# Coder-Yu/QRec

Hardware: AMD Instinct MI355X
Metric: BPR triplet-updates/sec (higher is better)
Workload: dtype f32

## Files before the change

qrec_amd/csrc/reduce.hip:

```cpp
#include "common.h"

using namespace qrec;

namespace {

template <typename T, typename V4>
__global__ __launch_bounds__(256) void sumsq_kernel(const T *__restrict__ x, int64_t n_elems,
                                                    double *__restrict__ out) {
    double acc = 0.0;
    const int64_t n4 = n_elems >> 2;
    const V4 *x4 = reinterpret_cast<const V4 *>(x);
    for (int64_t k = (int64_t)blockIdx.x * blockDim.x + threadIdx.x; k < n4;
         k += (int64_t)gridDim.x * blockDim.x) {
        const V4 v = x4[k];
        acc += (double)v.x * v.x + (double)v.y * v.y + (double)v.z * v.z + (double)v.w * v.w;
    }
    if (blockIdx.x == 0 && threadIdx.x < (n_elems & 3)) {
        const double v = (double)x[(n4 << 2) + threadIdx.x];
        acc += v * v;
    }
#pragma unroll
    for (int m = 32; m >= 1; m >>= 1) acc += __shfl_xor(acc, m, kWave);
    __shared__ double s_part[4];
    if ((threadIdx.x & 63) == 0) s_part[threadIdx.x >> 6] = acc;
    __syncthreads();
    if (threadIdx.x == 0) atomicAdd(out, s_part[0] + s_part[1] + s_part[2] + s_part[3]);
}

__device__ inline void driver_decide(double *__restrict__ stats, double *__restrict__ state, double regU, double regI,
                                     double max_lr, double tol, double *__restrict__ log, int64_t log_capacity) {
    const double nll = atomicAdd(stats + 0, 0.0);
    const double tp = stats[1], tq = stats[2];
    const double loss = nll + regU * tp + regI * tq;
    const double last = state[QREC_DRV_LAST_LOSS], lr_used = state[QREC_DRV_LR];
    const int64_t epoch = (int64_t)state[QREC_DRV_EPOCHS] + 1;
    double lr = lr_used;
    const bool finite = loss == loss && fabs(loss) <= 1.79769313486231570e308;
    const bool converged = finite && fabs(last - loss) < tol;
    if (finite && !converged) {
        if (epoch > 1) lr *= fabs(last) > fabs(loss) ? 1.05 : 0.5;
        if (max_lr > 0.0 && lr > max_lr) lr = max_lr;
    }
    state[QREC_DRV_LR] = lr;
    state[QREC_DRV_LAST_LOSS] = loss;
    state[QREC_DRV_EPOCHS] = (double)epoch;
    state[QREC_DRV_CONVERGED] = converged ? 1.0 : 0.0;
    state[QREC_DRV_FAILED] = finite ? 0.0 : 1.0;
    if (log && epoch <= log_capacity) {
        double *e = log + (epoch - 1) * QREC_DRV_LOG_WORDS;
        e[0] = loss; e[1] = lr_used; e[2] = nll; e[3] = last - loss; e[4] = tp; e[5] = tq;
    }
    stats[0] = 0.0;
}

template <typename T, typename V4>
__device__ inline double block_sumsq(const T *__restrict__ x, int64_t n_elems, double *s_part) {
    double acc = 0.0;
    const int64_t n4 = n_elems >> 2;
    const V4 *x4 = reinterpret_cast<const V4 *>(x);
    for (int64_t k = (int64_t)blockIdx.x * blockDim.x + threadIdx.x; k < n4; k += (int64_t)gridDim.x * blockDim.x) {
        const V4 v = x4[k];
        acc += (double)v.x * v.x + (double)v.y * v.y + (double)v.z * v.z + (double)v.w * v.w;
    }
#pragma unroll
    for (int m = 32; m >= 1; m >>= 1) acc += __shfl_xor(acc, m, kWave);
    __syncthreads();
    if ((threadIdx.x & 63) == 0) s_part[threadIdx.x >> 6] = acc;
    __syncthreads();
    return s_part[0] + s_part[1] + s_part[2] + s_part[3];
}

template <typename T, typename V4>
__global__ __launch_bounds__(256) void epoch_close_kernel(const T *__restrict__ P, int64_t p_elems,
                                                          const T *__restrict__ Q, int64_t q_elems,
                                                          double *__restrict__ stats, double *__restrict__ state,
                                                          double regU, double regI, double max_lr, double tol,
                                                          double *__restrict__ log, int64_t log_capacity, int decide) {
    if (state && (state[QREC_DRV_CONVERGED] != 0.0 || state[QREC_DRV_FAILED] != 0.0)) return;
    __shared__ double s_part[4];
    __shared__ bool s_last;
    const double sp = block_sumsq<T, V4>(P, p_elems, s_part);
    const double sq = block_sumsq<T, V4>(Q, q_elems, s_part);
    double *part = stats + QREC_STATS_PARTIALS;
    unsigned int *ticket = reinterpret_cast<unsigned int *>(stats + 3);
    if (threadIdx.x == 0) {
        __hip_atomic_store(part + 2 * blockIdx.x, sp, __ATOMIC_RELAXED, __HIP_MEMORY_SCOPE_AGENT);
        __hip_atomic_store(part + 2 * blockIdx.x + 1, sq, __ATOMIC_RELAXED, __HIP_MEMORY_SCOPE_AGENT);
        __threadfence();
        s_last = atomicAdd(ticket, 1u) == gridDim.x - 1;
    }
    __syncthreads();
    if (!s_last) return;
    __threadfence();
    double tp = 0.0, tq = 0.0;
    for (unsigned b = threadIdx.x; b < gridDim.x; b += blockDim.x) {
        tp += __hip_atomic_load(part + 2 * b, __ATOMIC_RELAXED, __HIP_MEMORY_SCOPE_AGENT);
        tq += __hip_atomic_load(part + 2 * b + 1, __ATOMIC_RELAXED, __HIP_MEMORY_SCOPE_AGENT);
    }
#pragma unroll
    for (int m = 32; m >= 1; m >>= 1) { tp += __shfl_xor(tp, m, kWave); tq += __shfl_xor(tq, m, kWave); }
    __shared__ double s_tot[2][4];
    if ((threadIdx.x & 63) == 0) { s_tot[0][threadIdx.x >> 6] = tp; s_tot[1][threadIdx.x >> 6] = tq; }
    __syncthreads();
    if (threadIdx.x != 0) return;
    tp = s_tot[0][0] + s_tot[0][1] + s_tot[0][2] + s_tot[0][3];
    tq = s_tot[1][0] + s_tot[1][1] + s_tot[1][2] + s_tot[1][3];
    if (!(decide & 2)) stats[1] = tp;
    if (!(decide & 4)) stats[2] = tq;
    *ticket = 0u;
    if (decide & 1) driver_decide(stats, state, regU, regI, max_lr, tol, log, log_capacity);
}

__global__ void epoch_decide_kernel(double *__restrict__ stats, double *__restrict__ state, double regU, double regI,
                                    double max_lr, double tol, double *__restrict__ log, int64_t log_capacity) {
    if (state[QREC_DRV_CONVERGED] != 0.0 || state[QREC_DRV_FAILED] != 0.0) return;
    driver_decide(stats, state, regU, regI, max_lr, tol, log, log_capacity);
}


__device__ inline bool last_block_total(double mine, int lane_of_pair, double *__restrict__ stats, double *total) {
    __shared__ bool s_last;
    __shared__ double s_tot[4];
    double *part = stats + QREC_STATS_PARTIALS;
    unsigned int *ticket = reinterpret_cast<unsigned int *>(stats + 3);
    if (threadIdx.x == 0) {
        __hip_atomic_store(part + 2 * blockIdx.x + lane_of_pair, mine, __ATOMIC_RELAXED, __HIP_MEMORY_SCOPE_AGENT);
        __threadfence();
        s_last = atomicAdd(ticket, 1u) == gridDim.x - 1;
    }
    __syncthreads();
    if (!s_last) return false;
    __threadfence();
    double t = 0.0;
    for (unsigned b = threadIdx.x; b < gridDim.x; b += blockDim.x)
        t += __hip_atomic_load(part + 2 * b + lane_of_pair, __ATOMIC_RELAXED, __HIP_MEMORY_SCOPE_AGENT);
#pragma unroll
    for (int m = 32; m >= 1; m >>= 1) t += __shfl_xor(t, m, kWave);
    if ((threadIdx.x & 63) == 0) s_tot[threadIdx.x >> 6] = t;
    __syncthreads();
    if (threadIdx.x != 0) return false;
    *total = s_tot[0] + s_tot[1] + s_tot[2] + s_tot[3];
    *ticket = 0u;
    return true;
}

__global__ __launch_bounds__(256) void dist_pre_kernel(const float *__restrict__ P, int64_t p_elems, const float4 *__restrict__ Q,
                                                       const float4 *__restrict__ start, float4 *__restrict__ delta,
                                                       int64_t q4, double *__restrict__ stats, const double *__restrict__ state) {
    if (state && (state[QREC_DRV_CONVERGED] != 0.0 || state[QREC_DRV_FAILED] != 0.0)) return;
    __shared__ double s_part[4];
    for (int64_t k = (int64_t)blockIdx.x * blockDim.x + threadIdx.x; k < q4; k += (int64_t)gridDim.x * blockDim.x) {
        const float4 a = Q[k], b = start[k];
        delta[k] = make_float4(a.x - b.x, a.y - b.y, a.z - b.z, a.w - b.w);
    }
    const double sp = block_sumsq<float, float4>(P, p_elems, s_part);
    double total;
    if (last_block_total(sp, 0, stats, &total)) stats[1] = total;
}

__global__ __launch_bounds__(256) void dist_post_kernel(float4 *__restrict__ Q, float4 *__restrict__ start,
                                                        const float4 *__restrict__ delta, int64_t q4, double *__restrict__ stats,
                                                        double *__restrict__ state, double regU, double regI, double max_lr,
                                                        double tol, double *__restrict__ log, int64_t log_capacity) {
    if (state[QREC_DRV_CONVERGED] != 0.0 || state[QREC_DRV_FAILED] != 0.0) return;
    double acc = 0.0;
    for (int64_t k = (int64_t)blockIdx.x * blockDim.x + threadIdx.x; k < q4; k += (int64_t)gridDim.x * blockDim.x) {
        const float4 s = start[k], d = delta[k];
        const float4 r = make_float4(s.x + d.x, s.y + d.y, s.z + d.z, s.w + d.w);
        start[k] = r;
        Q[k] = r;
        acc += (double)r.x * r.x + (double)r.y * r.y + (double)r.z * r.z + (double)r.w * r.w;
    }
#pragma unroll
    for (int m = 32; m >= 1; m >>= 1) acc += __shfl_xor(acc, m, kWave);
    __shared__ double s_part[4];
    if ((threadIdx.x & 63) == 0) s_part[threadIdx.x >> 6] = acc;
    __syncthreads();
    const double sq = s_part[0] + s_part[1] + s_part[2] + s_part[3];
    double total;
    if (last_block_total(sq, 1, stats, &total)) {
        stats[2] = total;
        driver_decide(stats, state, regU, regI, max_lr, tol, log, log_capacity);
    }
}

}

namespace {
int launch_epoch_close(const void *d_P, int64_t p_rows, const void *d_Q, int64_t q_rows, int dtype, int32_t ld,
                       double *d_stats, double *d_state, double regU, double regI, double max_lr, double tol,
                       double *d_log, int64_t log_capacity, int decide, hipStream_t st) {
    const int64_t pe = p_rows * (int64_t)ld, qe = q_rows * (int64_t)ld;
    int64_t blocks = ((pe > qe ? pe : qe) / 4 + 255) / 256;
    if (blocks > QREC_STATS_MAX_BLOCKS) blocks = QREC_STATS_MAX_BLOCKS;
    if (blocks < 1) blocks = 1;
    if (dtype == QREC_F32)
        hipLaunchKernelGGL((epoch_close_kernel<float, float4>), dim3((unsigned)blocks), dim3(256), 0, st, (const float *)d_P, pe,
                           (const float *)d_Q, qe, d_stats, d_state, regU, regI, max_lr, tol, d_log, log_capacity, decide);
    else
        hipLaunchKernelGGL((epoch_close_kernel<double, double4>), dim3((unsigned)blocks), dim3(256), 0, st, (const double *)d_P, pe,
                           (const double *)d_Q, qe, d_stats, d_state, regU, regI, max_lr, tol, d_log, log_capacity, decide);
    QREC_LAUNCH_CHECK();
    return QREC_OK;
}
}

extern "C" int qrec_epoch_close(const void *d_P, int64_t p_rows, const void *d_Q, int64_t q_rows, int dtype, int32_t ld,
                                double *d_stats, double *d_state, double regU, double regI, double max_lr,
                                double tol, double *d_log, int64_t log_capacity, void *stream) {
    QREC_REQUIRE(d_P && d_Q && d_stats && d_state && p_rows >= 0 && q_rows >= 0 && ld >= 4 && ld % 4 == 0,
                 "qrec_epoch_close: bad arguments");
    QREC_REQUIRE(dtype == QREC_F32 || dtype == QREC_F64, "qrec_epoch_close: bad dtype %d", dtype);
    QREC_REQUIRE(log_capacity == 0 || d_log, "qrec_epoch_close: log capacity without a log");
    return launch_epoch_close(d_P, p_rows, d_Q, q_rows, dtype, ld, d_stats, d_state, regU, regI, max_lr, tol, d_log,
                              log_capacity, 1, as_stream(stream));
}

extern "C" int qrec_epoch_sums(const void *d_P, int64_t p_rows, const void *d_Q, int64_t q_rows, int dtype, int32_t ld,
                               double *d_stats, const double *d_state, void *stream) {
    QREC_REQUIRE(d_P && d_Q && d_stats && p_rows >= 0 && q_rows >= 0 && ld >= 4 && ld % 4 == 0, "qrec_epoch_sums: bad arguments");
    QREC_REQUIRE(dtype == QREC_F32 || dtype == QREC_F64, "qrec_epoch_sums: bad dtype %d", dtype);
    return launch_epoch_close(d_P, p_rows, d_Q, q_rows, dtype, ld, d_stats, const_cast<double *>(d_state), 0, 0, 0, 0,
                              nullptr, 0, 0, as_stream(stream));
}
extern "C" int qrec_epoch_sum_table(const void *d_X, int64_t rows, int dtype, int32_t ld, double *d_stats, int slot,
                                    const double *d_state, void *stream) {
    QREC_REQUIRE(d_X && d_stats && rows >= 0 && ld >= 4 && ld % 4 == 0, "qrec_epoch_sum_table: bad arguments");
    QREC_REQUIRE(dtype == QREC_F32 || dtype == QREC_F64, "qrec_epoch_sum_table: bad dtype %d", dtype);
    QREC_REQUIRE(slot == 1 || slot == 2, "qrec_epoch_sum_table: slot must be 1 (sum P*P) or 2 (sum Q*Q)");
    return slot == 1 ? launch_epoch_close(d_X, rows, d_X, 0, dtype, ld, d_stats, const_cast<double *>(d_state), 0, 0, 0, 0, nullptr,
                                          0, 4, as_stream(stream))
                     : launch_epoch_close(d_X, 0, d_X, rows, dtype, ld, d_stats, const_cast<double *>(d_state), 0, 0, 0, 0, nullptr,
                                          0, 2, as_stream(stream));
}
extern "C" int qrec_epoch_decide(double *d_stats, double *d_state, double regU, double regI, double max_lr, double tol,
                                 double *d_log, int64_t log_capacity, void *stream) {
    QREC_REQUIRE(d_stats && d_state, "qrec_epoch_decide: null argument");
    QREC_REQUIRE(log_capacity == 0 || d_log, "qrec_epoch_decide: log capacity without a log");
    hipLaunchKernelGGL(epoch_decide_kernel, dim3(1), dim3(1), 0, as_stream(stream), d_stats, d_state, regU, regI, max_lr, tol,
                       d_log, log_capacity);
    QREC_LAUNCH_CHECK();
    return QREC_OK;
}

extern "C" int qrec_sumsq(const void *d_x, int dtype, int64_t rows, int32_t d, int32_t ld,
                          double *d_out, void *stream) {
    QREC_REQUIRE(d_out && rows >= 0 && d >= 1 && ld >= d, "qrec_sumsq: bad arguments");
    QREC_REQUIRE(dtype == QREC_F32 || dtype == QREC_F64, "qrec_sumsq: bad dtype %d", dtype);
    hipStream_t st = as_stream(stream);
    QREC_HIP_CHECK(hipMemsetAsync(d_out, 0, sizeof(double), st));
    if (rows == 0) return QREC_OK;
    QREC_REQUIRE(d_x, "qrec_sumsq: null table");
    const int64_t n = rows * (int64_t)ld;
    int64_t blocks = (n / 4 + 255) / 256;
    if (blocks > 1024) blocks = 1024;
    if (blocks < 1) blocks = 1;
    if (dtype == QREC_F32)
        hipLaunchKernelGGL((sumsq_kernel<float, float4>), dim3((unsigned)blocks), dim3(256), 0, st,
                           (const float *)d_x, n, d_out);
    else
        hipLaunchKernelGGL((sumsq_kernel<double, double4>), dim3((unsigned)blocks), dim3(256), 0, st,
                           (const double *)d_x, n, d_out);
    QREC_LAUNCH_CHECK();
    return QREC_OK;
}

extern "C" int qrec_dist_epoch_pre(const float *d_P, int64_t p_rows, int32_t ld, const float *d_Q, const float *d_Q_start,
                                   float *d_delta, int64_t q_rows, double *d_stats, const double *d_state, void *stream) {
    QREC_REQUIRE(d_P && d_Q && d_Q_start && d_delta && d_stats && p_rows >= 0 && q_rows >= 0 && ld >= 4 && ld % 4 == 0,
                 "qrec_dist_epoch_pre: bad arguments");
    const int64_t pe = p_rows * (int64_t)ld, q4 = q_rows * (int64_t)ld / 4;
    int64_t blocks = ((pe / 4 > q4 ? pe / 4 : q4) + 255) / 256;
    if (blocks > QREC_STATS_MAX_BLOCKS) blocks = QREC_STATS_MAX_BLOCKS;
    if (blocks < 1) blocks = 1;
    hipLaunchKernelGGL(dist_pre_kernel, dim3((unsigned)blocks), dim3(256), 0, as_stream(stream), d_P, pe, (const float4 *)d_Q,
                       (const float4 *)d_Q_start, (float4 *)d_delta, q4, d_stats, d_state);
    QREC_LAUNCH_CHECK();
    return QREC_OK;
}

extern "C" int qrec_dist_epoch_post(float *d_Q, float *d_Q_start, const float *d_delta, int64_t q_rows, int32_t ld,
                                    double *d_stats, double *d_state, double regU, double regI, double max_lr, double tol,
                                    double *d_log, int64_t log_capacity, void *stream) {
    QREC_REQUIRE(d_Q && d_Q_start && d_delta && d_stats && d_state && q_rows >= 0 && ld >= 4 && ld % 4 == 0,
                 "qrec_dist_epoch_post: bad arguments");
    QREC_REQUIRE(log_capacity == 0 || d_log, "qrec_dist_epoch_post: log capacity without a log");
    const int64_t q4 = q_rows * (int64_t)ld / 4;
    int64_t blocks = (q4 + 255) / 256;
    if (blocks > QREC_STATS_MAX_BLOCKS) blocks = QREC_STATS_MAX_BLOCKS;
    if (blocks < 1) blocks = 1;
    hipLaunchKernelGGL(dist_post_kernel, dim3((unsigned)blocks), dim3(256), 0, as_stream(stream), (float4 *)d_Q, (float4 *)d_Q_start,
                       (const float4 *)d_delta, q4, d_stats, d_state, regU, regI, max_lr, tol, d_log, log_capacity);
    QREC_LAUNCH_CHECK();
    return QREC_OK;
}
```

Baseline: 2.085 billion.

## Batch loads in reduction kernels and streamline last-block finalization

Rewrites the sum-of-squares, epoch-close and distributed pre/post kernels around a batched streaming loop that issues eight vector loads per thread before consuming them. P and Q are reduced in a single fused index space instead of two sequential passes. The grid is sized by the combined element count. Finalization now runs in one wave with DPP wave sums and readfirstlane instead of shared-memory barriers, and the driver state loads are issued alongside the partial loads. This targets memory latency and synchronization overhead in the per-epoch reductions, at the cost of more registers per thread and more complex code. It relies on wave_sum_dpp and f32x4 from common.h and on the block-count cap being exactly 256.

Result: no change. 2.103 billion, median of 4 (+0.9%).

```diff
diff --git a/qrec_amd/csrc/reduce.hip b/qrec_amd/csrc/reduce.hip
--- a/qrec_amd/csrc/reduce.hip
+++ b/qrec_amd/csrc/reduce.hip
@@ -4,36 +4,103 @@
 
 namespace {
 
+constexpr int kBatch = 8;
+constexpr int kBlock = 256;
+
+template <typename V4>
+__device__ inline double sumsq4(const V4 &v) {
+    return (double)v.x * v.x + (double)v.y * v.y + (double)v.z * v.z + (double)v.w * v.w;
+}
+
+typedef double f64x4 __attribute__((ext_vector_type(4)));
+struct F4Pair { f32x4 a, b; };
+
+__device__ inline void pin(f32x4 &v) { asm volatile("" : "+v"(v)); }
+__device__ inline void pin(f64x4 &v) { asm volatile("" : "+v"(v)); }
+__device__ inline void pin(F4Pair &v) { pin(v.a); pin(v.b); }
+
+template <typename Load, typename Use>
+__device__ inline void stream_batches(int64_t n, Load load, Use use) {
+    const int64_t stride = (int64_t)gridDim.x * kBlock;
+    for (int64_t base = (int64_t)blockIdx.x * kBlock + threadIdx.x; base < n; base += kBatch * stride) {
+        decltype(load(base)) v[kBatch];
+#pragma unroll
+        for (int j = 0; j < kBatch; j++) {
+            const int64_t k = base + j * stride;
+            v[j] = load(k < n ? k : n - 1);
+        }
+        asm volatile("" ::: "memory");
+#pragma unroll
+        for (int j = 0; j < kBatch; j++) pin(v[j]);
+#pragma unroll
+        for (int j = 0; j < kBatch; j++) {
+            const int64_t k = base + j * stride;
+            use(k, v[j], k < n);
+        }
+    }
+}
+
 template <typename T, typename V4>
-__global__ __launch_bounds__(256) void sumsq_kernel(const T *__restrict__ x, int64_t n_elems,
+__device__ inline void stream_sumsq2(const T *__restrict__ P, int64_t p_elems, const T *__restrict__ Q, int64_t q_elems,
+                                     double &sp, double &sq) {
+    const int64_t p4 = p_elems >> 2, q4 = q_elems >> 2;
+    const V4 *P4 = reinterpret_cast<const V4 *>(P), *Q4 = reinterpret_cast<const V4 *>(Q);
+    double ap = 0.0, aq = 0.0;
+    stream_batches(
+        p4 + q4, [=](int64_t k) { return *(k < p4 ? P4 + k : Q4 + (k - p4)); },
+        [&](int64_t k, const V4 &v, bool live) {
+            const double s = sumsq4(v);
+            ap += live && k < p4 ? s : 0.0;
+            aq += live && k >= p4 ? s : 0.0;
+        });
+    sp = ap; sq = aq;
+}
+
+__device__ inline void block_sum2_to_wave0(double &a, double &b, double *s_part) {
+    a = wave_sum_dpp(a); b = wave_sum_dpp(b);
+    if ((threadIdx.x & 63) == 0) { s_part[threadIdx.x >> 6] = a; s_part[4 + (threadIdx.x >> 6)] = b; }
+    __syncthreads();
+    a = s_part[0] + s_part[1] + s_part[2] + s_part[3];
+    b = s_part[4] + s_part[5] + s_part[6] + s_part[7];
+}
+
+template <typename T, typename V4>
+__global__ __launch_bounds__(kBlock) void sumsq_kernel(const T *__restrict__ x, int64_t n_elems,
                                                     double *__restrict__ out) {
-    double acc = 0.0;
     const int64_t n4 = n_elems >> 2;
     const V4 *x4 = reinterpret_cast<const V4 *>(x);
-    for (int64_t k = (int64_t)blockIdx.x * blockDim.x + threadIdx.x; k < n4;
-         k += (int64_t)gridDim.x * blockDim.x) {
-        const V4 v = x4[k];
-        acc += (double)v.x * v.x + (double)v.y * v.y + (double)v.z * v.z + (double)v.w * v.w;
-    }
+    double acc = 0.0, none = 0.0;
+    stream_batches(
+        n4, [=](int64_t k) { return x4[k]; }, [&](int64_t, const V4 &v, bool live) { acc += live ? sumsq4(v) : 0.0; });
     if (blockIdx.x == 0 && threadIdx.x < (n_elems & 3)) {
         const double v = (double)x[(n4 << 2) + threadIdx.x];
         acc += v * v;
     }
-#pragma unroll
-    for (int m = 32; m >= 1; m >>= 1) acc += __shfl_xor(acc, m, kWave);
-    __shared__ double s_part[4];
-    if ((threadIdx.x & 63) == 0) s_part[threadIdx.x >> 6] = acc;
-    __syncthreads();
-    if (threadIdx.x == 0) atomicAdd(out, s_part[0] + s_part[1] + s_part[2] + s_part[3]);
-}
-
-__device__ inline void driver_decide(double *__restrict__ stats, double *__restrict__ state, double regU, double regI,
-                                     double max_lr, double tol, double *__restrict__ log, int64_t log_capacity) {
-    const double nll = atomicAdd(stats + 0, 0.0);
-    const double tp = stats[1], tq = stats[2];
+    __shared__ double s_part[8];
+    block_sum2_to_wave0(acc, none, s_part);
+    if (threadIdx.x == 0) atomicAdd(out, acc);
+}
+
+
+__device__ inline bool run_is_over(const double *__restrict__ state) {
+    const double c = state[QREC_DRV_CONVERGED], f = state[QREC_DRV_FAILED];
+    return (c != 0.0) | (f != 0.0);
+}
+
+struct DriverIn { double nll, tp, tq, lr, last, epochs; };
+
+__device__ inline void driver_fetch(double *__restrict__ stats, const double *__restrict__ state, DriverIn &in) {
+    in.lr = state[QREC_DRV_LR]; in.last = state[QREC_DRV_LAST_LOSS]; in.epochs = state[QREC_DRV_EPOCHS];
+    in.nll = 0.0;
+    if (threadIdx.x == 0) in.nll = atomicAdd(stats + 0, 0.0);
+}
+
+__device__ inline void driver_decide(const DriverIn &in, double *__restrict__ stats, double *__restrict__ state, double regU,
+                                     double regI, double max_lr, double tol, double *__restrict__ log, int64_t log_capacity) {
+    const double nll = in.nll, tp = in.tp, tq = in.tq;
     const double loss = nll + regU * tp + regI * tq;
-    const double last = state[QREC_DRV_LAST_LOSS], lr_used = state[QREC_DRV_LR];
-    const int64_t epoch = (int64_t)state[QREC_DRV_EPOCHS] + 1;
+    const double last = in.last, lr_used = in.lr;
+    const int64_t epoch = (int64_t)in.epochs + 1;
     double lr = lr_used;
     const bool finite = loss == loss && fabs(loss) <= 1.79769313486231570e308;
     const bool converged = finite && fabs(last - loss) < tol;
@@ -53,135 +120,121 @@
     stats[0] = 0.0;
 }
 
+template <int HAVE, typename Fetch>
+__device__ inline bool last_block_totals(double sp, double sq, double *__restrict__ stats, double &tp, double &tq, Fetch fetch) {
+    static_assert(QREC_STATS_MAX_BLOCKS == 4 * kWave, "one wave reads four partials per lane");
+    double *part = stats + QREC_STATS_PARTIALS;
+    unsigned int *ticket = reinterpret_cast<unsigned int *>(stats + 3);
+    int last = 0;
+    if (threadIdx.x == 0) {
+        if (HAVE & 1) __hip_atomic_store(part + 2 * blockIdx.x, sp, __ATOMIC_RELAXED, __HIP_MEMORY_SCOPE_AGENT);
+        if (HAVE & 2) __hip_atomic_store(part + 2 * blockIdx.x + 1, sq, __ATOMIC_RELAXED, __HIP_MEMORY_SCOPE_AGENT);
+        asm volatile("s_waitcnt vmcnt(0)" ::: "memory");
+        last = atomicAdd(ticket, 1u) == gridDim.x - 1;
+    }
+    if (!__builtin_amdgcn_readfirstlane(last)) return false;
+    double a[4], b[4];
+#pragma unroll
+    for (int w = 0; w < 4; w++) {
+        const unsigned blk = w * kWave + threadIdx.x;
+        const double *p = part + 2 * (blk < gridDim.x ? blk : 0u);
+        a[w] = HAVE & 1 ? __hip_atomic_load(p, __ATOMIC_RELAXED, __HIP_MEMORY_SCOPE_AGENT) : 0.0;
+        b[w] = HAVE & 2 ? __hip_atomic_load(p + 1, __ATOMIC_RELAXED, __HIP_MEMORY_SCOPE_AGENT) : 0.0;
+    }
+    fetch();
+    double ta = 0.0, tb = 0.0;
+#pragma unroll
+    for (int w = 0; w < 4; w++) {
+        const bool live = w * kWave + threadIdx.x < gridDim.x;
+        ta += live ? a[w] : 0.0; tb += live ? b[w] : 0.0;
+    }
+    tp = wave_sum_dpp(ta); tq = wave_sum_dpp(tb);
+    return true;
+}
+
 template <typename T, typename V4>
-__device__ inline double block_sumsq(const T *__restrict__ x, int64_t n_elems, double *s_part) {
-    double acc = 0.0;
-    const int64_t n4 = n_elems >> 2;
-    const V4 *x4 = reinterpret_cast<const V4 *>(x);
-    for (int64_t k = (int64_t)blockIdx.x * blockDim.x + threadIdx.x; k < n4; k += (int64_t)gridDim.x * blockDim.x) {
-        const V4 v = x4[k];
-        acc += (double)v.x * v.x + (double)v.y * v.y + (double)v.z * v.z + (double)v.w * v.w;
-    }
-#pragma unroll
-    for (int m = 32; m >= 1; m >>= 1) acc += __shfl_xor(acc, m, kWave);
-    __syncthreads();
-    if ((threadIdx.x & 63) == 0) s_part[threadIdx.x >> 6] = acc;
-    __syncthreads();
-    return s_part[0] + s_part[1] + s_part[2] + s_part[3];
-}
-
-template <typename T, typename V4>
-__global__ __launch_bounds__(256) void epoch_close_kernel(const T *__restrict__ P, int64_t p_elems,
+__global__ __launch_bounds__(kBlock) void epoch_close_kernel(const T *__restrict__ P, int64_t p_elems,
                                                           const T *__restrict__ Q, int64_t q_elems,
                                                           double *__restrict__ stats, double *__restrict__ state,
                                                           double regU, double regI, double max_lr, double tol,
                                                           double *__restrict__ log, int64_t log_capacity, int decide) {
-    if (state && (state[QREC_DRV_CONVERGED] != 0.0 || state[QREC_DRV_FAILED] != 0.0)) return;
-    __shared__ double s_part[4];
-    __shared__ bool s_last;
-    const double sp = block_sumsq<T, V4>(P, p_elems, s_part);
-    const double sq = block_sumsq<T, V4>(Q, q_elems, s_part);
-    double *part = stats + QREC_STATS_PARTIALS;
-    unsigned int *ticket = reinterpret_cast<unsigned int *>(stats + 3);
-    if (threadIdx.x == 0) {
-        __hip_atomic_store(part + 2 * blockIdx.x, sp, __ATOMIC_RELAXED, __HIP_MEMORY_SCOPE_AGENT);
-        __hip_atomic_store(part + 2 * blockIdx.x + 1, sq, __ATOMIC_RELAXED, __HIP_MEMORY_SCOPE_AGENT);
-        __threadfence();
-        s_last = atomicAdd(ticket, 1u) == gridDim.x - 1;
-    }
-    __syncthreads();
-    if (!s_last) return;
-    __threadfence();
-    double tp = 0.0, tq = 0.0;
-    for (unsigned b = threadIdx.x; b < gridDim.x; b += blockDim.x) {
-        tp += __hip_atomic_load(part + 2 * b, __ATOMIC_RELAXED, __HIP_MEMORY_SCOPE_AGENT);
-        tq += __hip_atomic_load(part + 2 * b + 1, __ATOMIC_RELAXED, __HIP_MEMORY_SCOPE_AGENT);
-    }
-#pragma unroll
-    for (int m = 32; m >= 1; m >>= 1) { tp += __shfl_xor(tp, m, kWave); tq += __shfl_xor(tq, m, kWave); }
-    __shared__ double s_tot[2][4];
-    if ((threadIdx.x & 63) == 0) { s_tot[0][threadIdx.x >> 6] = tp; s_tot[1][threadIdx.x >> 6] = tq; }
-    __syncthreads();
+    if (state && run_is_over(state)) return;
+    __shared__ double s_part[8];
+    double sp, sq;
+    stream_sumsq2<T, V4>(P, p_elems, Q, q_elems, sp, sq);
+    block_sum2_to_wave0(sp, sq, s_part);
+    if (threadIdx.x >= kWave) return;
+    DriverIn in;
+    if (!last_block_totals<3>(sp, sq, stats, in.tp, in.tq, [&] { if (decide & 1) driver_fetch(stats, state, in); })) return;
     if (threadIdx.x != 0) return;
-    tp = s_tot[0][0] + s_tot[0][1] + s_tot[0][2] + s_tot[0][3];
-    tq = s_tot[1][0] + s_tot[1][1] + s_tot[1][2] + s_tot[1][3];
-    if (!(decide & 2)) stats[1] = tp;
-    if (!(decide & 4)) stats[2] = tq;
-    *ticket = 0u;
-    if (decide & 1) driver_decide(stats, state, regU, regI, max_lr, tol, log, log_capacity);
+    if (!(decide & 2)) stats[1] = in.tp;
+    if (!(decide & 4)) stats[2] = in.tq;
+    *reinterpret_cast<unsigned int *>(stats + 3) = 0u;
+    if (decide & 1) driver_decide(in, stats, state, regU, regI, max_lr, tol, log, log_capacity);
 }
 
 __global__ void epoch_decide_kernel(double *__restrict__ stats, double *__restrict__ state, double regU, double regI,
                                     double max_lr, double tol, double *__restrict__ log, int64_t log_capacity) {
-    if (state[QREC_DRV_CONVERGED] != 0.0 || state[QREC_DRV_FAILED] != 0.0) return;
-    driver_decide(stats, state, regU, regI, max_lr, tol, log, log_capacity);
-}
-
-
-__device__ inline bool last_block_total(double mine, int lane_of_pair, double *__restrict__ stats, double *total) {
-    __shared__ bool s_last;
-    __shared__ double s_tot[4];
-    double *part = stats + QREC_STATS_PARTIALS;
-    unsigned int *ticket = reinterpret_cast<unsigned int *>(stats + 3);
-    if (threadIdx.x == 0) {
-        __hip_atomic_store(part + 2 * blockIdx.x + lane_of_pair, mine, __ATOMIC_RELAXED, __HIP_MEMORY_SCOPE_AGENT);
-        __threadfence();
-        s_last = atomicAdd(ticket, 1u) == gridDim.x - 1;
-    }
-    __syncthreads();
-    if (!s_last) return false;
-    __threadfence();
-    double t = 0.0;
-    for (unsigned b = threadIdx.x; b < gridDim.x; b += blockDim.x)
-        t += __hip_atomic_load(part + 2 * b + lane_of_pair, __ATOMIC_RELAXED, __HIP_MEMORY_SCOPE_AGENT);
-#pragma unroll
-    for (int m = 32; m >= 1; m >>= 1) t += __shfl_xor(t, m, kWave);
-    if ((threadIdx.x & 63) == 0) s_tot[threadIdx.x >> 6] = t;
-    __syncthreads();
-    if (threadIdx.x != 0) return false;
-    *total = s_tot[0] + s_tot[1] + s_tot[2] + s_tot[3];
-    *ticket = 0u;
-    return true;
-}
-
-__global__ __launch_bounds__(256) void dist_pre_kernel(const float *__restrict__ P, int64_t p_elems, const float4 *__restrict__ Q,
+    if (run_is_over(state)) return;
+    DriverIn in;
+    driver_fetch(stats, state, in);
+    in.tp = stats[1]; in.tq = stats[2];
+    driver_decide(in, stats, state, regU, regI, max_lr, tol, log, log_capacity);
+}
+
+
+__global__ __launch_bounds__(kBlock) void dist_pre_kernel(const float *__restrict__ P, int64_t p_elems, const float4 *__restrict__ Q,
                                                        const float4 *__restrict__ start, float4 *__restrict__ delta,
                                                        int64_t q4, double *__restrict__ stats, const double *__restrict__ state) {
-    if (state && (state[QREC_DRV_CONVERGED] != 0.0 || state[QREC_DRV_FAILED] != 0.0)) return;
-    __shared__ double s_part[4];
-    for (int64_t k = (int64_t)blockIdx.x * blockDim.x + threadIdx.x; k < q4; k += (int64_t)gridDim.x * blockDim.x) {
-        const float4 a = Q[k], b = start[k];
-        delta[k] = make_float4(a.x - b.x, a.y - b.y, a.z - b.z, a.w - b.w);
-    }
-    const double sp = block_sumsq<float, float4>(P, p_elems, s_part);
+    if (state && run_is_over(state)) return;
+    __shared__ double s_part[8];
+    const f32x4 *P4 = reinterpret_cast<const f32x4 *>(P), *Q4 = reinterpret_cast<const f32x4 *>(Q),
+                *S4 = reinterpret_cast<const f32x4 *>(start);
+    f32x4 *D4 = reinterpret_cast<f32x4 *>(delta);
+    double sp = 0.0, none = 0.0;
+    stream_batches(
+        q4 + (p_elems >> 2),
+        [=](int64_t k) {
+            const f32x4 *pa = k < q4 ? Q4 + k : P4 + (k - q4), *pb = k < q4 ? S4 + k : pa;
+            return F4Pair{*pa, *pb};
+        },
+        [&](int64_t k, const F4Pair &v, bool live) {
+            if (live && k < q4) D4[k] = v.a - v.b;
+            sp += live && k >= q4 ? sumsq4(v.a) : 0.0;
+        });
+    block_sum2_to_wave0(sp, none, s_part);
+    if (threadIdx.x >= kWave) return;
     double total;
-    if (last_block_total(sp, 0, stats, &total)) stats[1] = total;
-}
-
-__global__ __launch_bounds__(256) void dist_post_kernel(float4 *__restrict__ Q, float4 *__restrict__ start,
+    if (last_block_totals<1>(sp, 0.0, stats, total, none, [] {}) && threadIdx.x == 0) {
+        stats[1] = total;
+        *reinterpret_cast<unsigned int *>(stats + 3) = 0u;
+    }
+}
+
+__global__ __launch_bounds__(kBlock) void dist_post_kernel(float4 *__restrict__ Q, float4 *__restrict__ start,
                                                         const float4 *__restrict__ delta, int64_t q4, double *__restrict__ stats,
                                                         double *__restrict__ state, double regU, double regI, double max_lr,
                                                         double tol, double *__restrict__ log, int64_t log_capacity) {
-    if (state[QREC_DRV_CONVERGED] != 0.0 || state[QREC_DRV_FAILED] != 0.0) return;
-    double acc = 0.0;
-    for (int64_t k = (int64_t)blockIdx.x * blockDim.x + threadIdx.x; k < q4; k += (int64_t)gridDim.x * blockDim.x) {
-        const float4 s = start[k], d = delta[k];
-        const float4 r = make_float4(s.x + d.x, s.y + d.y, s.z + d.z, s.w + d.w);
-        start[k] = r;
-        Q[k] = r;
-        acc += (double)r.x * r.x + (double)r.y * r.y + (double)r.z * r.z + (double)r.w * r.w;
-    }
-#pragma unroll
-    for (int m = 32; m >= 1; m >>= 1) acc += __shfl_xor(acc, m, kWave);
-    __shared__ double s_part[4];
-    if ((threadIdx.x & 63) == 0) s_part[threadIdx.x >> 6] = acc;
-    __syncthreads();
-    const double sq = s_part[0] + s_part[1] + s_part[2] + s_part[3];
-    double total;
-    if (last_block_total(sq, 1, stats, &total)) {
-        stats[2] = total;
-        driver_decide(stats, state, regU, regI, max_lr, tol, log, log_capacity);
-    }
+    if (run_is_over(state)) return;
+    __shared__ double s_part[8];
+    f32x4 *Q4 = reinterpret_cast<f32x4 *>(Q), *S4 = reinterpret_cast<f32x4 *>(start);
+    const f32x4 *D4 = reinterpret_cast<const f32x4 *>(delta);
+    double sq = 0.0, none = 0.0;
+    stream_batches(
+        q4, [=](int64_t k) { return F4Pair{S4[k], D4[k]}; },
+        [&](int64_t k, const F4Pair &v, bool live) {
+            const f32x4 r = v.a + v.b;
+            if (live) { S4[k] = r; Q4[k] = r; }
+            sq += live ? sumsq4(r) : 0.0;
+        });
+    block_sum2_to_wave0(sq, none, s_part);
+    if (threadIdx.x >= kWave) return;
+    DriverIn in;
+    if (!last_block_totals<2>(0.0, sq, stats, none, in.tq, [&] { driver_fetch(stats, state, in); in.tp = stats[1]; })) return;
+    if (threadIdx.x != 0) return;
+    stats[2] = in.tq;
+    *reinterpret_cast<unsigned int *>(stats + 3) = 0u;
+    driver_decide(in, stats, state, regU, regI, max_lr, tol, log, log_capacity);
 }
 
 }
@@ -191,14 +244,14 @@
                        double *d_stats, double *d_state, double regU, double regI, double max_lr, double tol,
                        double *d_log, int64_t log_capacity, int decide, hipStream_t st) {
     const int64_t pe = p_rows * (int64_t)ld, qe = q_rows * (int64_t)ld;
-    int64_t blocks = ((pe > qe ? pe : qe) / 4 + 255) / 256;
+    int64_t blocks = (pe / 4 + qe / 4 + kBlock - 1) / kBlock;
     if (blocks > QREC_STATS_MAX_BLOCKS) blocks = QREC_STATS_MAX_BLOCKS;
     if (blocks < 1) blocks = 1;
     if (dtype == QREC_F32)
-        hipLaunchKernelGGL((epoch_close_kernel<float, float4>), dim3((unsigned)blocks), dim3(256), 0, st, (const float *)d_P, pe,
+        hipLaunchKernelGGL((epoch_close_kernel<float, f32x4>), dim3((unsigned)blocks), dim3(kBlock), 0, st, (const float *)d_P, pe,
                            (const float *)d_Q, qe, d_stats, d_state, regU, regI, max_lr, tol, d_log, log_capacity, decide);
     else
-        hipLaunchKernelGGL((epoch_close_kernel<double, double4>), dim3((unsigned)blocks), dim3(256), 0, st, (const double *)d_P, pe,
+        hipLaunchKernelGGL((epoch_close_kernel<double, f64x4>), dim3((unsigned)blocks), dim3(kBlock), 0, st, (const double *)d_P, pe,
                            (const double *)d_Q, qe, d_stats, d_state, regU, regI, max_lr, tol, d_log, log_capacity, decide);
     QREC_LAUNCH_CHECK();
     return QREC_OK;
@@ -252,14 +305,14 @@
     if (rows == 0) return QREC_OK;
     QREC_REQUIRE(d_x, "qrec_sumsq: null table");
     const int64_t n = rows * (int64_t)ld;
-    int64_t blocks = (n / 4 + 255) / 256;
+    int64_t blocks = (n / 4 + kBlock - 1) / kBlock;
     if (blocks > 1024) blocks = 1024;
     if (blocks < 1) blocks = 1;
     if (dtype == QREC_F32)
-        hipLaunchKernelGGL((sumsq_kernel<float, float4>), dim3((unsigned)blocks), dim3(256), 0, st,
+        hipLaunchKernelGGL((sumsq_kernel<float, f32x4>), dim3((unsigned)blocks), dim3(kBlock), 0, st,
                            (const float *)d_x, n, d_out);
     else
-        hipLaunchKernelGGL((sumsq_kernel<double, double4>), dim3((unsigned)blocks), dim3(256), 0, st,
+        hipLaunchKernelGGL((sumsq_kernel<double, f64x4>), dim3((unsigned)blocks), dim3(kBlock), 0, st,
                            (const double *)d_x, n, d_out);
     QREC_LAUNCH_CHECK();
     return QREC_OK;
@@ -270,10 +323,10 @@
     QREC_REQUIRE(d_P && d_Q && d_Q_start && d_delta && d_stats && p_rows >= 0 && q_rows >= 0 && ld >= 4 && ld % 4 == 0,
                  "qrec_dist_epoch_pre: bad arguments");
     const int64_t pe = p_rows * (int64_t)ld, q4 = q_rows * (int64_t)ld / 4;
-    int64_t blocks = ((pe / 4 > q4 ? pe / 4 : q4) + 255) / 256;
+    int64_t blocks = (pe / 4 + q4 + kBlock - 1) / kBlock;
     if (blocks > QREC_STATS_MAX_BLOCKS) blocks = QREC_STATS_MAX_BLOCKS;
     if (blocks < 1) blocks = 1;
-    hipLaunchKernelGGL(dist_pre_kernel, dim3((unsigned)blocks), dim3(256), 0, as_stream(stream), d_P, pe, (const float4 *)d_Q,
+    hipLaunchKernelGGL(dist_pre_kernel, dim3((unsigned)blocks), dim3(kBlock), 0, as_stream(stream), d_P, pe, (const float4 *)d_Q,
                        (const float4 *)d_Q_start, (float4 *)d_delta, q4, d_stats, d_state);
     QREC_LAUNCH_CHECK();
     return QREC_OK;
@@ -286,10 +339,10 @@
                  "qrec_dist_epoch_post: bad arguments");
     QREC_REQUIRE(log_capacity == 0 || d_log, "qrec_dist_epoch_post: log capacity without a log");
     const int64_t q4 = q_rows * (int64_t)ld / 4;
-    int64_t blocks = (q4 + 255) / 256;
+    int64_t blocks = (q4 + kBlock - 1) / kBlock;
     if (blocks > QREC_STATS_MAX_BLOCKS) blocks = QREC_STATS_MAX_BLOCKS;
     if (blocks < 1) blocks = 1;
-    hipLaunchKernelGGL(dist_post_kernel, dim3((unsigned)blocks), dim3(256), 0, as_stream(stream), (float4 *)d_Q, (float4 *)d_Q_start,
+    hipLaunchKernelGGL(dist_post_kernel, dim3((unsigned)blocks), dim3(kBlock), 0, as_stream(stream), (float4 *)d_Q, (float4 *)d_Q_start,
                        (const float4 *)d_delta, q4, d_stats, d_state, regU, regI, max_lr, tol, d_log, log_capacity);
     QREC_LAUNCH_CHECK();
     return QREC_OK;
```
